# BenLangmead/bowtie2

Hardware: NVIDIA H100
Metric: Mreads/s (higher is better)
Workload: dtype u64 popcount (FM rank) + s16x2 DPX (DP)

## Files before the change

### bowtie2_b200/csrc/dp_kernels.cu

```cuda
#include "fm_device.cuh"
#include "dp_device.cuh"

#define DP_NEG (-(1 << 28))
#define DP_BIG (1 << 20)

__host__ __device__ __forceinline__ size_t dp_smem_per_warp(int maxCol) { return ((size_t)maxCol * 7 + 16 + 15) & ~(size_t)15; }

__device__ __forceinline__ int dp_max(int a, int b) { return a > b ? a : b; }

template <int R>
__device__ __forceinline__ void dp_backtrace_all(const DpLaunch &L, const bt2g_scoring &sc, const bt2g_dp_problem &p, uint64_t w,
                                                 const uint8_t *rs, const uint8_t *rq, int rdlen, const uint8_t *refw,
                                                 uint8_t *codes, bt2g_dp_cand *cands, int ncand, bt2g_dp_summary *summ,
                                                 int lane, bool local) {
	const int rdgapo = sc.rdgap_const + sc.rdgap_linear, rdgape = sc.rdgap_linear;
	const int rfgapo = sc.rfgap_const + sc.rfgap_linear, rfgape = sc.rfgap_linear;
	int SQ = rdlen >> 4; if(SQ == 0) SQ = 1;
	bt2g_dp_aln *alns = L.alns + w * (uint64_t)L.maxAlns;
	uint8_t *ops = L.ops + w * (uint64_t)L.maxAlns * L.maxOps;
	int naln = 0, flags = 0;
	auto cell = [&](int rr, int cc) -> uint8_t * { int k = rr / R; return codes + ((size_t)(cc + k) * 32 + k) * R + (rr - k * R); };
	for(int ci = 0; ci < ncand; ci++) {
		int row = cands[ci].row, col = cands[ci].col;
		const int startRow = row;
// ... 531 lines not shown
					if(c > 3) c = 5;
					bar = (i < sc.gapbar) || (rdlen[x] - 1 - i < sc.gapbar);
				}
				v[x][0] = c; v[x][1] = mm; v[x][2] = np;
				v[x][3] = bar ? -DPX_BIG : -rfgapo; v[x][4] = bar ? -DPX_BIG : -rfgape; v[x][5] = bar ? -DPX_BIG : -rdgapo;
			}
			rcP[r] = dpx_pack(v[0][0], v[1][0]); mmpP[r] = dpx_pack(v[0][1], v[1][1]); npnP[r] = dpx_pack(v[0][2], v[1][2]);
			nrfoP[r] = dpx_pack(v[0][3], v[1][3]); nrfeP[r] = dpx_pack(v[0][4], v[1][4]); nrdoP[r] = dpx_pack(v[0][5], v[1][5]);
		}
		const int lastLane0 = (rdlen[0] - 1) / R, lastLane1 = (rdlen[1] - 1) / R;
		const int lastLaneMax = lastLane0 > lastLane1 ? lastLane0 : lastLane1;
		const uint32_t nfloorP = dpx_pack(-floorv[0], -floorv[1]);

		uint32_t Hleft[R], Earr[R];
#pragma unroll
		for(int r = 0; r < R; r++) { Hleft[r] = FLOORP; Earr[r] = FLOORP; }
		uint32_t botH = FLOORP, botF = FLOORP, prevInH = FLOORP;
		const int nsteps = ncolMax + lastLaneMax;
		const size_t P4 = (size_t)(L.maxCol + 32) * 128, P1 = (size_t)(L.maxCol + 32) * 32;
		uint8_t *w4A[R / 4 + 1], *w4B[R / 4 + 1], *w1A[R % 4 + 1], *w1B[R % 4 + 1];
#pragma unroll
		for(int g = 0; g < R / 4; g++) { w4A[g] = hb[0] + g * P4 + (size_t)lane * 4; w4B[g] = hb[1] + g * P4 + (size_t)lane * 4; }
#pragma unroll
		for(int g = 0; g < R % 4; g++) { w1A[g] = hb[0] + (R / 4) * P4 + g * P1 + lane; w1B[g] = hb[1] + (R / 4) * P4 + g * P1 + lane; }
		for(int t = 0; t < nsteps; t++) {
			uint32_t inH = __shfl_up_sync(0xffffffffu, botH, 1);
			uint32_t inF = __shfl_up_sync(0xffffffffu, botF, 1);
			if(lane == 0) { inH = FLOORP; inF = FLOORP; }
			const int j = t - lane;
			if(j >= 0 && j < ncolMax && lane <= lastLaneMax) {
				const uint32_t refcP = (uint32_t)refw[0][j] | ((uint32_t)refw[1][j] << 16);
				const uint32_t refNm = ((refcP >> 2) & ONEP) * 0xffffu;
				uint32_t diag = (lane == 0) ? 0u : prevInH;
				uint32_t upH = inH, upF = inF;
				uint32_t hs[DP_RP(R)];
#pragma unroll
				for(int r = R; r < DP_RP(R); r++) hs[r] = 0u;
#pragma unroll
				for(int r = 0; r < R; r++) {
					const uint32_t F = __viaddmax_s16x2(upF, nrfeP[r], __viaddmax_s16x2(upH, nrfoP[r], FLOORP));
					const uint32_t pen = dpx_sel(refNm, npnP[r], mmpP[r]);
					const uint32_t mmask = dpx_ne01(rcP[r], refcP) * 0xffffu;
					const uint32_t Hd = __viaddmax_s16x2(diag, dpx_sel(mmask, pen, bonusP), FLOORP);
					const uint32_t E = Earr[r];
					const uint32_t H = __vimax3_s16x2(Hd, E, F);
					Earr[r] = __viaddmax_s16x2(E, nrdeP, __viaddmax_s16x2(H, nrdoP[r], FLOORP));
					hs[r] = __viaddmax_s16x2(H, nfloorP, 0u);
					diag = Hleft[r]; Hleft[r] = H;
					upH = H; upF = F;
				}
				botH = upH; botF = upF;
				prevInH = inH;
#pragma unroll
				for(int q4 = 0; q4 < R / 4; q4++) {
					const uint32_t t01 = __byte_perm(hs[4 * q4], hs[4 * q4 + 1], 0x6240), t23 = __byte_perm(hs[4 * q4 + 2], hs[4 * q4 + 3], 0x6240);
					*reinterpret_cast<uint32_t *>(w4A[q4]) = __byte_perm(t01, t23, 0x5410);
					*reinterpret_cast<uint32_t *>(w4B[q4]) = __byte_perm(t01, t23, 0x7632);
				}
#pragma unroll
				for(int g = 0; g < R % 4; g++) {
					*w1A[g] = (uint8_t)(hs[(R / 4) * 4 + g] & 0xffu);
					*w1B[g] = (uint8_t)((hs[(R / 4) * 4 + g] >> 16) & 0xffu);
				}
			} else if(j >= ncolMax) {
				botH = FLOORP; botF = FLOORP;
			}
#pragma unroll
			for(int g = 0; g < R / 4; g++) { w4A[g] += 128; w4B[g] += 128; }
#pragma unroll
			for(int g = 0; g < R % 4; g++) { w1A[g] += 32; w1B[g] += 32; }
		}
		__syncwarp();
#pragma unroll
		for(int x = 0; x < 2; x++) {
			if(!live[x]) continue;
			const int lr = rdlen[x] - 1, kk = lr / R;
			for(int j = lane; j < ncol[x]; j += 32)
				lastH[x][j] = (int)hb[x][hb_index<R>(L.maxCol + 32, lr, j)] + floorv[x];
			dp_e2e_tail<R, true>(L, sc, p[x], w[x], rs[x], rq[x], rdlen[x], ncol[x], lastH[x], candCol[x], refw[x], hb[x], L.summ + w[x], lane,
			                     DpHbPlanes<R>{hb[x], L.maxCol + 32});
		}
	}
}

#define DP_BLK_ROWS (32 * DP_BLOCK_RPL)
#define DP_BLK_HEAD 64
#define DP_BLK_MAX (DP_BLK_HEAD / 4)
static_assert(16 * 32 <= DP_BLK_MAX * DP_BLK_ROWS, "the range table must cover reads of 32 x 16 rows");

#define DP_FILL_PAD 64
__host__ __device__ __forceinline__ size_t dp_fill_smem_per_warp(int maxCol, bool offdom) {
	const size_t win = ((size_t)maxCol + 15) & ~(size_t)15;
	return 2 * (win + 2 * DP_FILL_PAD) + DP_QPROF_BYTES(DP_BLOCK_RPL) + win * (offdom ? 4 : 8);
}

template <bool B> struct DpBool { static constexpr bool value = B; };

template <typename OFF, int R, bool OFFDOM>
__global__ void __launch_bounds__(128, 8) k_dp_fill_h(DevIndex<OFF> ix, bt2g_scoring sc, DpLaunch L, uint64_t chunkStart, uint64_t chunkMax) {
	constexpr int RPL = DP_BLOCK_RPL;
	static_assert(RPL == 1 || RPL == 2, "stores are one byte or one u16 per lane and problem");
	extern __shared__ uint8_t smem[];
	const int warpInBlock = threadIdx.x >> 5, lane = threadIdx.x & 31;
	const uint64_t slot = blockIdx.x * (uint64_t)(blockDim.x >> 5) + warpInBlock;
	const uint64_t nSlots = (uint64_t)gridDim.x * (blockDim.x >> 5);
	const uint64_t nAll = L.nDev ? (uint64_t)*L.nDev : L.n;
	if(chunkStart >= nAll) return;
	const uint64_t nProb = (nAll - chunkStart < chunkMax) ? nAll - chunkStart : chunkMax;
	const uint64_t nPairs = (nProb + 1) >> 1;
	const size_t win = ((size_t)L.maxCol + 15) & ~(size_t)15;
	uint8_t *sm0 = smem + (size_t)warpInBlock * dp_fill_smem_per_warp(L.maxCol, OFFDOM);
	uint8_t *refw[2] = {sm0 + DP_FILL_PAD, sm0 + win + 3 * DP_FILL_PAD}; uint8_t *hb[2];
	for(int k = lane; k < 2 * ((int)win + 2 * DP_FILL_PAD); k += 32) sm0[k] = 4;
	uint32_t *qprof = reinterpret_cast<uint32_t *>(sm0 + 2 * (win + 2 * DP_FILL_PAD));
	uint32_t *bnd = reinterpret_cast<uint32_t *>(sm0 + 2 * (win + 2 * DP_FILL_PAD) + DP_QPROF_BYTES(RPL));
	const int rdgapo = sc.rdgap_const + sc.rdgap_linear, rdgape = sc.rdgap_linear;
	const int rfgapo = sc.rfgap_const + sc.rfgap_linear, rfgape = sc.rfgap_linear;
	const int bonus = sc.match_bonus;
	const uint32_t FLOORP = OFFDOM ? L.zeroP : dpx_both(DPX_FLOOR);
	const uint32_t nrdeP = dpx_both(-rdgape);

	for(uint64_t pw = slot; pw < nPairs; pw += nSlots) {
		uint64_t w[2] = {2 * pw, 2 * pw + 1};
		bool live[2] = {true, w[1] < nProb};
		if(!live[1]) w[1] = w[0];
		bt2g_dp_problem p[2] = {L.probs[chunkStart + w[0]], L.probs[chunkStart + w[1]]};
		hb[0] = L.codes + w[0] * L.codeStride; hb[1] = L.codes + w[1] * L.codeStride;
		uint64_t ro[2]; int rdlen[2], ncol[2], floorv[2];
		__syncwarp();
#pragma unroll
		for(int x = 0; x < 2; x++) {
			ro[x] = L.roff[p[x].read_idx];
			rdlen[x] = (int)(L.roff[p[x].read_idx + 1] - L.roff[p[x].read_idx]);
			ncol[x] = (int)(p[x].refr - p[x].refl + 1);
			floorv[x] = p[x].minsc - bonus - 1;
			if(ncol[x] <= 0 || ncol[x] > L.maxCol || rdlen[x] > 32 * R || rdlen[x] <= 0 ||
			   (int64_t)bonus * rdlen[x] - floorv[x] > 127 || floorv[x] < -DPX_LIMIT) {
				if(live[x] && lane == 0) {
					bt2g_dp_summary *sm = L.summ + chunkStart + w[x];
					sm->found = 0; sm->best = DP_NEG; sm->ncand = 0; sm->naln = 0; sm->flags = BT2G_DP_FLAG_BADSHAPE;
				}
				live[x] = false;
			}
		}
		if(!live[0] && !live[1]) continue;
		if(!live[0]) { p[0] = p[1]; ro[0] = ro[1]; rdlen[0] = rdlen[1]; ncol[0] = ncol[1]; floorv[0] = floorv[1]; }
		if(!live[1]) { p[1] = p[0]; ro[1] = ro[0]; rdlen[1] = rdlen[0]; ncol[1] = ncol[0]; floorv[1] = floorv[0]; }
		const int ncolMax = ncol[0] > ncol[1] ? ncol[0] : ncol[1];
#pragma unroll
		for(int x = 0; x < 2; x++) {
			ref_window<OFF>(ix, p[x].tidx, p[x].refl, ncol[x], refw[x], lane);
			for(int k = ncol[x] + lane; k < ncolMax; k += 32) refw[x][k] = 4;
		}
		__syncwarp();
		const int rdMax = rdlen[0] > rdlen[1] ? rdlen[0] : rdlen[1];
		const int nblk = (rdMax + DP_BLK_ROWS - 1) / DP_BLK_ROWS;
		const uint32_t nfloorP = dpx_pack(-floorv[0], -floorv[1]);
		uint32_t off = DP_BLK_HEAD;
		int plo = 0, phi = -1;

		for(int b = 0; b < nblk; b++) {
			int lo = 0, bLast = -1, nst = 0;
			if(OFFDOM && b > 0) {
				int first = -1;
				for(int c0 = plo; c0 <= phi; c0 += 32) {
					const int c = c0 + lane;
					const uint32_t m = __ballot_sync(0xffffffffu, c <= phi && bnd[c] != 0u);
					if(m) { if(first < 0) first = c0 + __ffs(m) - 1; bLast = c0 + 31 - __clz(m); }
				}
				lo = first < 0 ? 0 : first;
			}
			if(!OFFDOM || b == 0 || bLast >= 0) {
				uint32_t nrfoP[RPL], nrfeP[RPL], nrdoP[RPL];
#pragma unroll
				for(int r = 0; r < RPL; r++) {
					int v[2][3];
#pragma unroll
					for(int x = 0; x < 2; x++) {
						const int i = b * DP_BLK_ROWS + lane * RPL + r;
						bool bar = true;
						int c = 5, mm = -DPX_BIG, np = -DPX_BIG;
						if(i < rdlen[x]) {
							const int pos = p[x].fw ? i : rdlen[x] - 1 - i;
							c = L.seq[ro[x] + pos];
							c = p[x].fw ? c : (c > 3 ? 4 : 3 - c);
							int q = (int)L.qual[ro[x] + pos] - 33;
							q = q < 0 ? 0 : (q > 63 ? 63 : q);
							np = -(int)sc.npen[q];
							mm = c > 3 ? np : -(int)sc.mmpen[q];
							if(c > 3) c = 5;
							bar = (i < sc.gapbar) || (rdlen[x] - 1 - i < sc.gapbar);
						}
#pragma unroll
						for(int rf = 0; rf < 5; rf++) {
							const uint32_t pv = (uint32_t)(uint16_t)(int16_t)(rf > 3 ? np : (c == rf ? bonus : mm));
							uint32_t &q = qprof[(rf * RPL + r) * 32 + lane];
							q = x == 0 ? pv : (q | (pv << 16));
						}
						v[x][0] = bar ? -DPX_BIG : -rfgapo; v[x][1] = bar ? -DPX_BIG : -rfgape; v[x][2] = bar ? -DPX_BIG : -rdgapo;
					}
					nrfoP[r] = dpx_pack(v[0][0], v[1][0]); nrfeP[r] = dpx_pack(v[0][1], v[1][1]); nrdoP[r] = dpx_pack(v[0][2], v[1][2]);
				}
				int lastLane = (rdMax - 1 - b * DP_BLK_ROWS) / RPL;
				if(lastLane > 31) lastLane = 31;
				const bool keepBottom = b + 1 < nblk;

				const int nsteps = ncolMax - lo + lastLane;
				const int lim = lane <= lastLane ? ncolMax - lo : 0;
				auto sweep = [&](auto top) -> int {
					constexpr bool TOP = decltype(top)::value;
					constexpr int SG = 4;
					uint32_t Hleft[RPL], Earr[RPL];
#pragma unroll
					for(int r = 0; r < RPL; r++) { Hleft[r] = FLOORP; Earr[r] = FLOORP; }
					uint32_t botH = FLOORP, botF = FLOORP, prevInH = FLOORP;
					uint8_t *dA = hb[0] + off + lane * RPL, *dB = hb[1] + off + lane * RPL;
					for(int t0 = 0; t0 < nsteps; t0 += SG, dA += SG * 32 * RPL, dB += SG * 32 * RPL) {
#pragma unroll
						for(int u = 0; u < SG; u++) {
							const int t = t0 + u;
							uint32_t inH = __shfl_up_sync(0xffffffffu, botH, 1);
							uint32_t inF = __shfl_up_sync(0xffffffffu, botF, 1);
							if(TOP) {
								if(lane == 0) { inH = FLOORP; inF = FLOORP; }
							} else {
								uint32_t bh = FLOORP, bf = FLOORP;
								if(lo + t <= phi) {
									if(OFFDOM) { const uint32_t e = bnd[lo + t]; bh = __byte_perm(e, 0u, 0x4140); bf = __byte_perm(e, 0u, 0x4342); }
									else { const uint2 e = reinterpret_cast<const uint2 *>(bnd)[lo + t]; bh = e.x; bf = e.y; }
								}
								if(lane == 0) { inH = bh; inF = bf; }
							}
							const bool on = (unsigned)(t - lane) < (unsigned)lim;
							if(OFFDOM || on) {
								const int j = lo + t - lane;
								const uint32_t *qa = qprof + (int)refw[0][j] * (RPL * 32) + lane, *qb = qprof + (int)refw[1][j] * (RPL * 32) + lane;
								uint32_t diag = (TOP && lane == 0) ? (OFFDOM ? nfloorP : 0u) : prevInH;
								uint32_t upH = inH, upF = inF;
								uint32_t hs[RPL];
#pragma unroll
								for(int r = 0; r < RPL; r++) {
									const uint32_t F = __viaddmax_s16x2(upF, nrfeP[r], __viaddmax_s16x2(upH, nrfoP[r], FLOORP));
									const uint32_t sP = (qa[r * 32] & 0x0000ffffu) | (qb[r * 32] & 0xffff0000u);
									const uint32_t Hd = __viaddmax_s16x2(diag, sP, FLOORP);
									const uint32_t E = Earr[r];
									const uint32_t H = __vimax3_s16x2(Hd, E, F);
									Earr[r] = __viaddmax_s16x2(E, nrdeP, __viaddmax_s16x2(H, nrdoP[r], FLOORP));
									hs[r] = OFFDOM ? H : __viaddmax_s16x2(H, nfloorP, 0u);
									diag = Hleft[r]; Hleft[r] = H;
									upH = H; upF = F;
								}
								botH = upH; botF = upF;
								prevInH = inH;
								if(OFFDOM || on) {
									if(RPL == 2) {
										const uint32_t w2 = __byte_perm(hs[0], hs[RPL - 1], 0x6240);
										*reinterpret_cast<uint16_t *>(dA + u * 32 * RPL) = (uint16_t)w2;
										*reinterpret_cast<uint16_t *>(dB + u * 32 * RPL) = (uint16_t)(w2 >> 16);
									} else {
										dA[u * 32 * RPL] = (uint8_t)hs[0]; dB[u * 32 * RPL] = (uint8_t)(hs[0] >> 16);
									}
									if(keepBottom && lane == 31 && on) {
										if(OFFDOM) bnd[j] = __byte_perm(botH, botF, 0x6420);
										else reinterpret_cast<uint2 *>(bnd)[j] = make_uint2(botH, botF);
									}
								}
							} else {
								botH = FLOORP; botF = FLOORP;
							}
						}
						if(!TOP && OFFDOM && lo + t0 + SG - 1 >= bLast) {
							uint32_t s = botH | botF | prevInH;
#pragma unroll
							for(int r = 0; r < RPL; r++) s |= Hleft[r] | Earr[r];
							if(!__any_sync(0xffffffffu, t0 + SG - 1 - lane < lim && s != 0u)) return t0 + SG < nsteps ? t0 + SG : nsteps;
						}
					}
					return nsteps;
				};
				nst = b == 0 ? sweep(DpBool<true>()) : sweep(DpBool<false>());
			}
			if(lane == 0) {
				reinterpret_cast<uint32_t *>(hb[0])[b] = (uint32_t)lo | ((uint32_t)nst << 16);
				reinterpret_cast<uint32_t *>(hb[1])[b] = (uint32_t)lo | ((uint32_t)nst << 16);
			}
			off += (uint32_t)nst * 32 * RPL;
			plo = lo; phi = lo + nst - 32;
			if(phi > ncolMax - 1) phi = ncolMax - 1;
			__syncwarp();
		}
	}
}

struct DpHbBlocks {
	uint8_t *hb; const uint2 *tab;
	__device__ __forceinline__ uint8_t *operator()(int rr, int cc) const {
		const int k = (rr % DP_BLK_ROWS) / DP_BLOCK_RPL;
		const uint2 e = tab[rr / DP_BLK_ROWS];
		const int st = cc - (int)(e.x & 0xffffu) + k;
		return (st >= k && st < (int)(e.x >> 16)) ? hb + e.y + ((size_t)st * 32 + k) * DP_BLOCK_RPL + rr % DP_BLOCK_RPL : nullptr;
	}
};

#define DP_TAIL_SMEM_PER_WARP(maxCol, R) (dp_smem_per_warp(maxCol) + DP_PROF_BYTES(R) + DP_BLK_MAX * sizeof(uint2))

template <typename OFF, int R>
__global__ void __launch_bounds__(256) k_dp_tail_h(DevIndex<OFF> ix, bt2g_scoring sc, DpLaunch L, uint64_t chunkStart, uint64_t chunkMax) {
	extern __shared__ uint8_t smem[];
	const int warpInBlock = threadIdx.x >> 5, lane = threadIdx.x & 31;
	const uint64_t nAll = L.nDev ? (uint64_t)*L.nDev : L.n;
	if(chunkStart >= nAll) return;
	const uint64_t nProb = (nAll - chunkStart < chunkMax) ? nAll - chunkStart : chunkMax;
	const size_t perWarp = DP_TAIL_SMEM_PER_WARP(L.maxCol, R);
	int32_t *lastH = reinterpret_cast<int32_t *>(smem + (size_t)warpInBlock * perWarp);
	uint16_t *candCol = reinterpret_cast<uint16_t *>(lastH + L.maxCol);
	uint8_t *refw = reinterpret_cast<uint8_t *>(candCol + L.maxCol);
	uint8_t *prof = smem + (size_t)warpInBlock * perWarp + dp_smem_per_warp(L.maxCol);
	uint2 *tab = reinterpret_cast<uint2 *>(prof + DP_PROF_BYTES(R));
	const int bonus = sc.match_bonus;
	const uint64_t nWarps = (uint64_t)gridDim.x * (blockDim.x >> 5);
	for(uint64_t wl = blockIdx.x * (uint64_t)(blockDim.x >> 5) + warpInBlock; wl < nProb; wl += nWarps) {
		const uint64_t w = chunkStart + wl;
		const bt2g_dp_problem p = L.probs[w];
		const uint8_t *rs = L.seq + L.roff[p.read_idx], *rq = L.qual + L.roff[p.read_idx];
		const int rdlen = (int)(L.roff[p.read_idx + 1] - L.roff[p.read_idx]);
		const int ncol = (int)(p.refr - p.refl + 1);
		const int floorv = p.minsc - bonus - 1;
		__syncwarp();
		if(ncol <= 0 || ncol > L.maxCol || rdlen > 32 * R || rdlen <= 0 || (int64_t)bonus * rdlen - floorv > 127 || floorv < -DPX_LIMIT) continue;
		uint8_t *hb = L.codes + wl * L.codeStride;
		const int nblk = (rdlen + DP_BLK_ROWS - 1) / DP_BLK_ROWS;
		const uint32_t e = lane < nblk ? reinterpret_cast<const uint32_t *>(hb)[lane] : 0u;
		const uint32_t bytes = (e >> 16) * (32 * DP_BLOCK_RPL);
		uint32_t incl = bytes;
#pragma unroll
		for(int o = 1; o < 32; o <<= 1) { const uint32_t v = __shfl_up_sync(0xffffffffu, incl, o); if(lane >= o) incl += v; }
		if(lane < nblk) tab[lane] = make_uint2(e, DP_BLK_HEAD + incl - bytes);
		ref_window<OFF>(ix, p.tidx, p.refl, ncol, refw, lane);
		for(int i = lane; i < rdlen; i += 32) {
			const int pos = p.fw ? i : rdlen - 1 - i;
			int c = rs[pos]; c = p.fw ? c : (c > 3 ? 4 : 3 - c);
			int q = (int)rq[pos] - 33; q = q < 0 ? 0 : (q > 63 ? 63 : q);
			prof[i] = (uint8_t)c; prof[rdlen + i] = sc.mmpen[q]; prof[2 * rdlen + i] = sc.npen[q];
		}
		__syncwarp();
		const DpHbBlocks cell{hb, tab};
		const int lr = rdlen - 1;
		for(int j = lane; j < ncol; j += 32) { const uint8_t *c = cell(lr, j); lastH[j] = (c ? (int)*c : 0) + floorv; }
		dp_e2e_tail<R, true>(L, sc, p, w, rs, rq, rdlen, ncol, lastH, candCol, refw, hb, L.summ + w, lane, cell, prof);
	}
}

template <typename Acc>
__device__ __forceinline__ void dp_backtrace_h(const DpLaunch &L, const bt2g_scoring &sc, const bt2g_dp_problem &p, uint64_t w,
                                               const uint8_t *rs, const uint8_t *rq, int rdlen, const uint8_t *refw,
                                               const Acc &cell, bt2g_dp_cand *cands, int ncand, bt2g_dp_summary *summ, int lane,
                                               const uint8_t *prof) {
	const int rdgapo = sc.rdgap_const + sc.rdgap_linear, rdgape = sc.rdgap_linear;
	const int rfgapo = sc.rfgap_const + sc.rfgap_linear, rfgape = sc.rfgap_linear;
	const int bonus = sc.match_bonus, gapbar = sc.gapbar;
	const int vmax = bonus * rdlen - (p.minsc - bonus - 1);
	bt2g_dp_aln *alns = L.alns + w * (uint64_t)L.maxAlns;
	uint8_t *ops = L.ops + w * (uint64_t)L.maxAlns * L.maxOps;
	int naln = 0, flags = 0;
	bool screened = false;
	auto cellv = [&](int rr, int cc) -> int { const uint8_t *c = cell(rr, cc); return c ? (int)*c : 0; };
	auto rdchar = [&](int rr) -> int { const int pos = p.fw ? rr : rdlen - 1 - rr; int c = rs[pos]; return p.fw ? c : (c > 3 ? 4 : 3 - c); };
	auto rdqual = [&](int rr) -> int { const int pos = p.fw ? rr : rdlen - 1 - rr; int q = (int)rq[pos] - 33; return q < 0 ? 0 : (q > 63 ? 63 : q); };
	auto inCore = [&](int dlo, int dhi) -> bool { return dhi >= p.corel && dlo <= p.corer; };
	for(int ci = 0; ci < ncand; ci++) {
		int row = cands[ci].row, col = cands[ci].col;
		const int startRow = row, origCol = col;
		uint8_t *o = ops + (size_t)naln * L.maxOps;
		const bool room = naln < L.maxAlns;
		int nops = 0, ns = 0, gaps = 0;
		bool fail = false, core = false, done = false, first = true, filtStart = false;
		while(!done && !fail) {
			const int wd = (ci > 0 && first) ? 8 : 32;
			const int rk = row - lane, ck = col - lane;
			const bool in = lane < wd && rk >= 0 && ck >= 0;
			uint8_t *cp = in ? cell(rk, ck) : nullptr;
			const int mine = in ? (cp ? (int)*cp : 0) : 0x80;
			const int v = mine & 0x7f;
			const int vn = __shfl_down_sync(0xffffffffu, v, 1);
			int sck = 0, refc = 4; bool isN = false, isMatch = false;
			if(in) {
				refc = refw[ck];
				if(prof) {
					const int c = prof[rk];
					isN = c > 3 || refc > 3;
					isMatch = !isN && c == refc;
					sck = isN ? -(int)prof[2 * rdlen + rk] : (isMatch ? bonus : -(int)prof[rdlen + rk]);
				} else {
					const int c = rdchar(rk), q = rdqual(rk);
					isN = c > 3 || refc > 3;
					isMatch = !isN && c == refc;
					sck = isN ? -(int)sc.npen[q] : (isMatch ? bonus : -(int)sc.mmpen[q]);
				}
			}
			const bool cont = lane < wd - 1 && !(mine & 0x80) && rk > 0 && ck > 0 && vn > 0 && v == vn + sck;
			const int run = __ffs(~__ballot_sync(0xffffffffu, cont)) - 1;
			if(run > 0) {
				first = false;
				const int diagi = col - row + p.triml;
				if(inCore(diagi, diagi)) core = true;
				if(lane < run) {
					const uint8_t op = (uint8_t)((isMatch ? BT2G_OP_MATCH : BT2G_OP_MM) | (refc << 2));
					if(room && nops + lane < L.maxOps) o[nops + lane] = op;
					if(cp) *cp = (uint8_t)(mine | 0x80);
				}
				ns += __popc(__ballot_sync(0xffffffffu, lane < run && isN));
				nops += run; row -= run; col -= run;
			}
			const int endBits = __shfl_sync(0xffffffffu, mine, run);
			if(run == wd - 1 && !(endBits & 0x80) && row > 0 && col > 0) { __syncwarp(); continue; }
			if(endBits & 0x80) {
				if(first) filtStart = true;
				fail = true; break;
			}
			first = false;
			if(lane == run && cp) *cp = (uint8_t)(mine | 0x80);
			{
				const int diagi = col - row + p.triml;
				if(inCore(diagi, diagi)) core = true;
			}
			if(row == 0) { done = true; break; }
			const int cur = endBits & 0x7f;
			__syncwarp();
			int klen = 0, gapKind = 0;
			if(row >= gapbar && rdlen - 1 - row >= gapbar) {
				for(int k0 = 0; k0 < row; k0 += 32) {
					if(vmax - rfgapo - k0 * rfgape < cur) break;
					const int k = k0 + lane + 1, r2 = row - k;
					bool ok = false;
					if(r2 >= 0 && row - k + 1 >= gapbar && vmax - rfgapo - (k - 1) * rfgape >= cur) {
						const int u = cellv(r2, col) & 0x7f;
						ok = u > 0 && u - rfgapo - (k - 1) * rfgape == cur;
					}
					const uint32_t mk = __ballot_sync(0xffffffffu, ok);
					if(mk) { klen = k0 + __ffs(mk); gapKind = 1; break; }
				}
				if(gapKind == 0) {
					for(int k0 = 0; k0 < col; k0 += 32) {
						if(vmax - rdgapo - k0 * rdgape < cur) break;
						const int k = k0 + lane + 1, c2 = col - k;
						bool ok = false;
						if(c2 >= 0 && vmax - rdgapo - (k - 1) * rdgape >= cur) {
							const int u = cellv(row, c2) & 0x7f;
							ok = u > 0 && u - rdgapo - (k - 1) * rdgape == cur;
						}
						const uint32_t mk = __ballot_sync(0xffffffffu, ok);
						if(mk) { klen = k0 + __ffs(mk); gapKind = 2; break; }
					}
				}
			}
			if(gapKind == 0) { fail = true; break; }
			for(int m0 = 1; m0 < klen && !fail; m0 += 32) {
				const int mth = m0 + lane;
				uint8_t *q2 = nullptr; int b = 0;
				if(mth < klen) { q2 = gapKind == 1 ? cell(row - mth, col) : cell(row, col - mth); b = q2 ? *q2 : 0; }
				const uint32_t vm = __ballot_sync(0xffffffffu, (b & 0x80) != 0);
				const int lim = vm ? __ffs(vm) - 1 : 32;
				if(q2 && lane < lim) *q2 = (uint8_t)(b | 0x80);
				if(vm) fail = true;
			}
			if(fail) break;
			{
				const int d0 = col - row + p.triml, ni = klen - 1;
				if(ni > 0 && (gapKind == 1 ? inCore(d0 + 1, d0 + ni) : inCore(d0 - ni, d0 - 1))) core = true;
			}
			if(room) {
				for(int k = lane; k < klen; k += 32) {
					const int idx = nops + k;
					if(idx < L.maxOps) o[idx] = gapKind == 1 ? (uint8_t)BT2G_OP_REFGAP : (uint8_t)(BT2G_OP_READGAP | (refw[col - k] << 2));
				}
			}
			nops += klen; gaps += klen;
			if(gapKind == 1) row -= klen; else col -= klen;
			__syncwarp();
		}
		if(filtStart) { if(lane == 0) cands[ci].fate = BT2G_CAND_FILT_START; continue; }
		if(!fail) {
			const int c = rdchar(row), refc = refw[col];
			const bool isN = c > 3 || refc > 3;
			ns += isN;
			const uint8_t op = (uint8_t)(((!isN && c == refc) ? BT2G_OP_MATCH : BT2G_OP_MM) | (refc << 2));
			if(!core) fail = true;
			else if(ns > p.nceil) fail = true;
			else {
				if(room && lane == 0 && nops < L.maxOps) o[nops] = op;
				nops++;
			}
		}
		const bool opOverflow = nops > L.maxOps;
		if(fail) { if(lane == 0) cands[ci].fate = BT2G_CAND_FAILED; continue; }
		if(lane == 0) cands[ci].fate = BT2G_CAND_SUCCEEDED;
		if(room) {
			int refns = 0;
			for(int k = col + lane; k <= origCol; k += 32) refns += refw[k] > 3;
			refns = __reduce_add_sync(0xffffffffu, refns);
			if(lane == 0) {
				bt2g_dp_aln &a = alns[naln];
				a.cand_idx = ci; a.score = cands[ci].score; a.ns = ns; a.gaps = gaps; a.col0 = col; a.row0 = row;
				a.trim_beg = 0; a.trim_end = rdlen - 1 - startRow; a.nops = nops;
				a.refns = refns;
			}
			if(opOverflow) flags |= BT2G_DP_FLAG_OPS_OVERFLOW;
		} else {
			flags |= BT2G_DP_FLAG_ALN_OVERFLOW;
		}
		naln++;
		if(naln == 1 && !screened && ci + 1 < ncand) {
			screened = true;
			bool needSeq = false;
			for(int base = ci + 1; base < ncand; base += 32) {
				const int cj = base + lane;
				int verdict = 0;
				if(cj < ncand) {
					int r2 = cands[cj].row, c2 = cands[cj].col;
					int b = cellv(r2, c2);
					if(b & 0x80) verdict = 1;
					else {
						for(int guard = 0; guard < 4 * rdlen + 8; guard++) {
							const int curv = b & 0x7f;
							if(r2 == 0) { verdict = 2; break; }
							if(c2 > 0) {
								const int pb = cellv(r2 - 1, c2 - 1), pv = pb & 0x7f;
								const int rf = refw[c2];
								int c, mm, np;
								if(prof) { c = prof[r2]; mm = prof[rdlen + r2]; np = prof[2 * rdlen + r2]; }
								else { c = rdchar(r2); const int q = rdqual(r2); mm = sc.mmpen[q]; np = sc.npen[q]; }
								const int sc2 = (c > 3 || rf > 3) ? -np : (c == rf ? bonus : -mm);
								if(pv > 0 && curv == pv + sc2) {
									if(pb & 0x80) break;
									r2--; c2--; b = pb;
									continue;
								}
							}
							if(r2 < gapbar || rdlen - 1 - r2 < gapbar) break;
							bool moved = false, dead = false, marked = false;
							for(int k = 1; k <= r2 && r2 - k + 1 >= gapbar && vmax - rfgapo - (k - 1) * rfgape >= curv; k++) {
								const int ub = cellv(r2 - k, c2), u = ub & 0x7f;
								if(u > 0 && u - rfgapo - (k - 1) * rfgape == curv) {
									if(marked || (ub & 0x80)) dead = true; else { r2 -= k; b = ub; moved = true; }
									break;
								}
								marked = marked || (ub & 0x80);
							}
							if(!moved && !dead) {
								marked = false;
								for(int k = 1; k <= c2 && vmax - rdgapo - (k - 1) * rdgape >= curv; k++) {
									const int ub = cellv(r2, c2 - k), u = ub & 0x7f;
									if(u > 0 && u - rdgapo - (k - 1) * rdgape == curv) {
										if(marked || (ub & 0x80)) dead = true; else { c2 -= k; b = ub; moved = true; }
										break;
									}
									marked = marked || (ub & 0x80);
								}
							}
							if(!moved) break;
						}
					}
				}
				if(__any_sync(0xffffffffu, verdict == 2)) { needSeq = true; break; }
				if(cj < ncand) cands[cj].fate = verdict == 1 ? BT2G_CAND_FILT_START : BT2G_CAND_FAILED;
			}
			__syncwarp();
			if(!needSeq) break;
		}
	}
	if(lane == 0) { summ->naln = naln; summ->flags |= flags; }
}

template <typename K>
static unsigned dp_resident_grid(K kernel, int threads, size_t smem, uint64_t numSlots, int warpsPerBlock) {
	int dev = 0, sms = 148, nb = 1;
	cudaGetDevice(&dev);
	cudaDeviceGetAttribute(&sms, cudaDevAttrMultiProcessorCount, dev);
	if(cudaOccupancyMaxActiveBlocksPerMultiprocessor(&nb, kernel, threads, smem) != cudaSuccess || nb < 1) nb = 1;
	uint64_t g = (uint64_t)nb * sms, cap = numSlots / warpsPerBlock;
	return (unsigned)(g < cap ? g : cap);
}

template <typename OFF, int R>
static void launch_dp_e2e_r(const DevIndex<OFF> &ix, const bt2g_scoring &sc, const DpLaunch &L, cudaStream_t st) {
	const int warpsPerBlock = 4;
	if(L.packed == 3) {
		int dev = 0, sms = 148; cudaGetDevice(&dev); cudaDeviceGetAttribute(&sms, cudaDevAttrMultiProcessorCount, dev);
		const size_t smF = (size_t)warpsPerBlock * dp_fill_smem_per_warp(L.maxCol, sc.match_bonus == 0);
		const size_t smT = (size_t)8 * DP_TAIL_SMEM_PER_WARP(L.maxCol, R);
		auto kfill = sc.match_bonus == 0 ? k_dp_fill_h<OFF, R, true> : k_dp_fill_h<OFF, R, false>;
		if(smF > 48 * 1024) cudaFuncSetAttribute(kfill, cudaFuncAttributeMaxDynamicSharedMemorySize, (int)smF);
		if(smT > 48 * 1024) cudaFuncSetAttribute(k_dp_tail_h<OFF, R>, cudaFuncAttributeMaxDynamicSharedMemorySize, (int)smT);
		int nbF = 1, nbT = 1;
		if(cudaOccupancyMaxActiveBlocksPerMultiprocessor(&nbF, kfill, warpsPerBlock * 32, smF) != cudaSuccess || nbF < 1) nbF = 1;
		if(cudaOccupancyMaxActiveBlocksPerMultiprocessor(&nbT, k_dp_tail_h<OFF, R>, 256, smT) != cudaSuccess || nbT < 1) nbT = 1;
		auto mark = [&]() { if(L.tev && L.tevN && *L.tevN < L.tevCap) cudaEventRecord(L.tev[(*L.tevN)++], st); };
		mark();
		for(uint64_t c0 = 0; c0 < L.n; c0 += L.chunk) {
			kfill<<<(unsigned)(nbF * sms), warpsPerBlock * 32, smF, st>>>(ix, sc, L, c0, L.chunk);
			mark();
			k_dp_tail_h<OFF, R><<<(unsigned)(nbT * sms), 256, smT, st>>>(ix, sc, L, c0, L.chunk);
			mark();
		}
	} else if(L.packed == 2) {
		const size_t smem = (size_t)warpsPerBlock * 2 * dp_smem_per_warp(L.maxCol);
		if(smem > 48 * 1024) cudaFuncSetAttribute(k_dp_e2e_h<OFF, R>, cudaFuncAttributeMaxDynamicSharedMemorySize, (int)smem);
		const unsigned grid = dp_resident_grid(k_dp_e2e_h<OFF, R>, warpsPerBlock * 32, smem, L.numSlots, warpsPerBlock);
		k_dp_e2e_h<OFF, R><<<grid, warpsPerBlock * 32, smem, st>>>(ix, sc, L);
	} else if(L.packed) {
		const size_t smem = (size_t)warpsPerBlock * 2 * dp_smem_per_warp(L.maxCol);
		if(smem > 48 * 1024) cudaFuncSetAttribute(k_dp_e2e_x2<OFF, R>, cudaFuncAttributeMaxDynamicSharedMemorySize, (int)smem);
		const unsigned grid = dp_resident_grid(k_dp_e2e_x2<OFF, R>, warpsPerBlock * 32, smem, L.numSlots, warpsPerBlock);
		k_dp_e2e_x2<OFF, R><<<grid, warpsPerBlock * 32, smem, st>>>(ix, sc, L);
	} else {
		const size_t smem = (size_t)warpsPerBlock * dp_smem_per_warp(L.maxCol);
		if(smem > 48 * 1024) cudaFuncSetAttribute(k_dp_e2e<OFF, R>, cudaFuncAttributeMaxDynamicSharedMemorySize, (int)smem);
		const unsigned grid = dp_resident_grid(k_dp_e2e<OFF, R>, warpsPerBlock * 32, smem, L.numSlots, warpsPerBlock);
		k_dp_e2e<OFF, R><<<grid, warpsPerBlock * 32, smem, st>>>(ix, sc, L);
	}
}

template <typename OFF>
int launch_dp_e2e(const DevIndex<OFF> &ix, const bt2g_scoring &sc, const DpLaunch &L, int maxRdLen, cudaStream_t st) {
	if(L.n == 0) return 0;
	switch(dp_rows_per_lane(maxRdLen, L.packed)) {
		case 4: launch_dp_e2e_r<OFF, 4>(ix, sc, L, st); break;
		case 5: launch_dp_e2e_r<OFF, 5>(ix, sc, L, st); break;
		case 6: launch_dp_e2e_r<OFF, 6>(ix, sc, L, st); break;
		case 8: launch_dp_e2e_r<OFF, 8>(ix, sc, L, st); break;
		case 10: launch_dp_e2e_r<OFF, 10>(ix, sc, L, st); break;
		case 12: launch_dp_e2e_r<OFF, 12>(ix, sc, L, st); break;
		case 16: launch_dp_e2e_r<OFF, 16>(ix, sc, L, st); break;
		default: return -1;
	}
	return 0;
}
template int launch_dp_e2e<uint32_t>(const DevIndex<uint32_t> &, const bt2g_scoring &, const DpLaunch &, int, cudaStream_t);
template int launch_dp_e2e<uint64_t>(const DevIndex<uint64_t> &, const bt2g_scoring &, const DpLaunch &, int, cudaStream_t);

template <typename OFF, int R>
__global__ void __launch_bounds__(128) k_dp_local(DevIndex<OFF> ix, bt2g_scoring sc, DpLaunch L) {
	extern __shared__ uint8_t smem[];
	const int warpInBlock = threadIdx.x >> 5, lane = threadIdx.x & 31;
	const uint64_t slot = blockIdx.x * (uint64_t)(blockDim.x >> 5) + warpInBlock;
	const uint64_t nSlots = (uint64_t)gridDim.x * (blockDim.x >> 5);
	const uint64_t nProb = L.nDev ? (uint64_t)*L.nDev : L.n;
	const size_t perWarp = dp_smem_per_warp(L.maxCol);
	int32_t *wsm = reinterpret_cast<int32_t *>(smem + (size_t)warpInBlock * perWarp);
	uint8_t *refw = reinterpret_cast<uint8_t *>(wsm + L.maxCol) + 2 * (size_t)L.maxCol;
	uint8_t *codes = L.codes + slot * L.codeStride;
	uint64_t *raw = L.rawKeys + slot * (uint64_t)L.maxRaw;
	const int rdgapo = sc.rdgap_const + sc.rdgap_linear, rdgape = sc.rdgap_linear;
	const int rfgapo = sc.rfgap_const + sc.rfgap_linear, rfgape = sc.rfgap_linear;
	const int bonus = sc.match_bonus;

	for(uint64_t w = slot; w < nProb; w += nSlots) {
		const bt2g_dp_problem p = L.probs[w];
		const uint8_t *rs = L.seq + L.roff[p.read_idx];
		const uint8_t *rq = L.qual + L.roff[p.read_idx];
		const int rdlen = (int)(L.roff[p.read_idx + 1] - L.roff[p.read_idx]);
		const int ncol = (int)(p.refr - p.refl + 1);
		bt2g_dp_summary *summ = L.summ + w;
		__syncwarp();
		if(ncol <= 0 || ncol + 1 > L.maxCol || rdlen > 32 * R || rdlen <= 0 || bonus <= 0) {
			if(lane == 0) { summ->found = 0; summ->best = DP_NEG; summ->ncand = 0; summ->naln = 0; summ->flags = BT2G_DP_FLAG_BADSHAPE; }
			continue;
		}
		for(int k = lane; k <= ncol; k += 32) refw[k] = (uint8_t)ref_base<OFF>(ix, p.tidx, p.refl + k);
		if(lane == 0) wsm[0] = 0;
		__syncwarp();

		int rc[R + 1], mmp[R], npn[R];
		bool bar[R];
#pragma unroll
		for(int r = 0; r <= R; r++) {
			int i = lane * R + r;
			int c = 6;
			if(i < rdlen) {
				int pos = p.fw ? i : rdlen - 1 - i;
				c = rs[pos];
				c = p.fw ? c : (c > 3 ? 4 : 3 - c);
				if(r < R) {
					int q = (int)rq[pos] - 33;
					q = q < 0 ? 0 : (q > 63 ? 63 : q);
					npn[r] = sc.npen[q];
					mmp[r] = c > 3 ? npn[r] : sc.mmpen[q];
					bar[r] = (i < sc.gapbar) || (rdlen - 1 - i < sc.gapbar);
				}
			} else if(r < R) { mmp[r] = 0; npn[r] = 0; bar[r] = true; }
			rc[r] = c;
		}
		const int lastLane = (rdlen - 1) / R;
		const int minrow = (int)(((int64_t)p.minsc + bonus - 1) / bonus) - 1;

		int Hleft[R], Earr[R], Eprev[R];
#pragma unroll
		for(int r = 0; r < R; r++) { Hleft[r] = 0; Earr[r] = 0; Eprev[r] = 0; }
		int botH = 0, botF = 0, prevInH = 0, lmax = 0;
		const int nsteps = ncol + lastLane;
		for(int t = 0; t < nsteps; t++) {
			int inH = __shfl_up_sync(0xffffffffu, botH, 1);
			int inF = __shfl_up_sync(0xffffffffu, botF, 1);
			if(lane == 0) { inH = 0; inF = 0; }
			const int j = t - lane;
			if(j >= 0 && j < ncol && lane <= lastLane) {
				const int refc = refw[j], refn = refw[j + 1];
				const bool refN = refc > 3;
				int diag = (lane == 0) ? 0 : prevInH;
				int upH = inH, upF = inF;
				uint32_t packed[(R + 3) / 4];
#pragma unroll
				for(int q4 = 0; q4 < (R + 3) / 4; q4++) packed[q4] = 0;
#pragma unroll
				for(int r = 0; r < R; r++) {
					const int i = lane * R + r;
					const int fo = upH - rfgapo, fe = upF - rfgape;
					int F = bar[r] ? 0 : dp_max(dp_max(fo, fe), 0);
					const int fsel = (upH > 0 && fo == F) ? 1 : ((upF > 0 && fe == F) ? 2 : 0);
					int s = (rc[r] == refc && !refN) ? bonus : -mmp[r];
					s = (refN || rc[r] > 3) ? -npn[r] : s;
					const int Hd = diag + s;
					const int E = Earr[r];
					const int H = dp_max(__vimax3_s32(Hd, E, F), 0);
					int hsel = 0;
					if(diag > 0 && H == Hd) hsel = 1;
					else if(!bar[r]) {
						if(upH > 0 && H == fo) hsel = 2;
						else if(upF > 0 && H == fe) hsel = 3;
						else if(Hleft[r] > 0 && H == Hleft[r] - rdgapo) hsel = 4;
						else if(Eprev[r] > 0 && H == Eprev[r] - rdgape) hsel = 5;
					}
					const int esel = (Hleft[r] > 0 && Hleft[r] - rdgapo == E) ? 1 : ((Eprev[r] > 0 && Eprev[r] - rdgape == E) ? 2 : 0);
					const uint32_t code = (uint32_t)(hsel | (esel << 3) | (fsel << 5));
					packed[r >> 2] |= code << ((r & 3) * 8);
					const int eo = bar[r] ? 0 : H - rdgapo, ee = E - rdgape;
					if(i < rdlen && i >= minrow && H >= p.minsc && rc[r] == refc && !(i < rdlen - 1 && rc[r + 1] == refn)) {
						const int pos = atomicAdd(&wsm[0], 1);
						if(pos < L.maxRaw) raw[pos] = ((uint64_t)(uint32_t)H << 32) | ((uint64_t)i << 16) | (uint64_t)j;
					}
					lmax = dp_max(lmax, i < rdlen ? H : 0);
					diag = Hleft[r]; Hleft[r] = H; Eprev[r] = E; Earr[r] = dp_max(dp_max(eo, ee), 0);
					upH = H; upF = F;
				}
				botH = upH; botF = upF;
				prevInH = inH;
				uint8_t *dst = codes + ((size_t)t * 32 + lane) * R;
				if(R == 4) *reinterpret_cast<uint32_t *>(dst) = packed[0];
				else if(R == 8) *reinterpret_cast<uint2 *>(dst) = make_uint2(packed[0], packed[1]);
				else {
#pragma unroll
					for(int q4 = 0; q4 < (R + 3) / 4; q4++) reinterpret_cast<uint32_t *>(dst)[q4] = packed[q4];
				}
			} else if(j >= ncol) {
				botH = 0; botF = 0;
			}
		}
		__syncwarp();
		int best = lmax;
#pragma unroll
		for(int o = 16; o > 0; o >>= 1) best = dp_max(best, __shfl_xor_sync(0xffffffffu, best, o));
		if(lane == 0) { summ->best = best; summ->flags = 0; summ->naln = 0; summ->ncand = 0; summ->found = 0; }
		if(best < p.minsc) continue;
		const int nrawAll = wsm[0];
		const int nraw = nrawAll < L.maxRaw ? nrawAll : L.maxRaw;
		bt2g_dp_cand *cands = L.cands + w * (uint64_t)L.maxCands;
		for(int a0 = 0; a0 < nraw; a0 += 32) {
			const int a = a0 + lane;
			if(a < nraw) {
				const uint64_t key = raw[a];
				int rank = 0;
				for(int k = 0; k < nraw; k++) rank += raw[k] > key;
				if(rank < L.maxCands) {
					cands[rank].score = (int32_t)(key >> 32); cands[rank].row = (int32_t)((key >> 16) & 0xffff);
					cands[rank].col = (int32_t)(key & 0xffff); cands[rank].fate = 0;
				}
			}
		}
		const int ncand = nraw < L.maxCands ? nraw : L.maxCands;
		if(lane == 0) {
			summ->ncand = nrawAll; summ->found = nrawAll > 0;
			if(nrawAll > L.maxCands || nrawAll > L.maxRaw) summ->flags |= BT2G_DP_FLAG_CAND_OVERFLOW;
		}
		__syncwarp();
		dp_backtrace_all<R>(L, sc, p, w, rs, rq, rdlen, refw, codes, cands, ncand, summ, lane, true);
	}
}

template <typename OFF>
int launch_dp_local(const DevIndex<OFF> &ix, const bt2g_scoring &sc, const DpLaunch &L, int maxRdLen, cudaStream_t st) {
	if(L.n == 0) return 0;
	const int warpsPerBlock = 4;
	const size_t perWarp = dp_smem_per_warp(L.maxCol);
	size_t smem = (size_t)warpsPerBlock * perWarp;
	unsigned grid = (unsigned)(L.numSlots / warpsPerBlock);
	if(maxRdLen <= 128) {
		if(smem > 48 * 1024) cudaFuncSetAttribute(k_dp_local<OFF, 4>, cudaFuncAttributeMaxDynamicSharedMemorySize, (int)smem);
		k_dp_local<OFF, 4><<<grid, warpsPerBlock * 32, smem, st>>>(ix, sc, L);
	} else if(maxRdLen <= 256) {
		if(smem > 48 * 1024) cudaFuncSetAttribute(k_dp_local<OFF, 8>, cudaFuncAttributeMaxDynamicSharedMemorySize, (int)smem);
		k_dp_local<OFF, 8><<<grid, warpsPerBlock * 32, smem, st>>>(ix, sc, L);
	} else if(maxRdLen <= 512) {
		if(smem > 48 * 1024) cudaFuncSetAttribute(k_dp_local<OFF, 16>, cudaFuncAttributeMaxDynamicSharedMemorySize, (int)smem);
		k_dp_local<OFF, 16><<<grid, warpsPerBlock * 32, smem, st>>>(ix, sc, L);
	} else {
		return -1;
	}
	return 0;
}
template int launch_dp_local<uint32_t>(const DevIndex<uint32_t> &, const bt2g_scoring &, const DpLaunch &, int, cudaStream_t);
template int launch_dp_local<uint64_t>(const DevIndex<uint64_t> &, const bt2g_scoring &, const DpLaunch &, int, cudaStream_t);
```

Baseline: 2.754.

## Rework DP tail kernel: warp-parallel candidate selection, dynamic work claiming, skip empty problems

New measurement: 2.800 (median of 6 runs). 1.02x the previous value.

```diff
diff --git a/bowtie2_b200/csrc/dp_kernels.cu b/bowtie2_b200/csrc/dp_kernels.cu
--- a/bowtie2_b200/csrc/dp_kernels.cu
+++ b/bowtie2_b200/csrc/dp_kernels.cu
@@ -857,52 +857,151 @@
 	}
 };
 
-#define DP_TAIL_SMEM_PER_WARP(maxCol, R) (dp_smem_per_warp(maxCol) + DP_PROF_BYTES(R) + DP_BLK_MAX * sizeof(uint2))
+__host__ __device__ __forceinline__ int dp_tail_key_cap(int maxCands, int maxCol) {
+	const int n = maxCands < maxCol ? maxCands : maxCol;
+	int c = 1;
+	while(c < n) c <<= 1;
+	return c;
+}
+__host__ __device__ __forceinline__ size_t dp_tail_win_bytes(int maxCol) { return ((size_t)maxCol + 15) & ~(size_t)15; }
+__host__ __device__ __forceinline__ size_t dp_tail_smem_per_warp(int maxCol, int maxCands, int R) {
+	return (dp_tail_win_bytes(maxCol) + DP_PROF_BYTES(R) + DP_BLK_MAX * sizeof(uint2) + (size_t)dp_tail_key_cap(maxCands, maxCol) * 4 + 15) &
+	       ~(size_t)15;
+}
+__host__ __device__ __forceinline__ unsigned *dp_tail_claim(const DpLaunch &L) { return reinterpret_cast<unsigned *>(L.codes + L.codeStride) - 1; }
+
+__device__ __forceinline__ int dp_tail_cands(const DpLaunch &L, const bt2g_dp_problem &p, const uint8_t *hb, const uint2 *tab, int rdlen,
+                                             int ncol, int floorv, uint32_t *keys, bt2g_dp_cand *cands, bt2g_dp_summary *summ, int lane) {
+	const int lr = rdlen - 1, k = (lr % DP_BLK_ROWS) / DP_BLOCK_RPL;
+	const uint2 e = tab[lr / DP_BLK_ROWS];
+	const int lo = (int)(e.x & 0xffffu), steps = (int)(e.x >> 16);
+	const int hi = lo + steps - k < ncol ? lo + steps - k : ncol;
+	const uint8_t *row = hb + e.y + (size_t)k * 33 * DP_BLOCK_RPL + lr % DP_BLOCK_RPL;
+	auto key = [&](int c) -> uint32_t { return c < hi ? (uint32_t)row[(size_t)(c - lo) * 32 * DP_BLOCK_RPL] << 16 | (uint32_t)c : 0u; };
+	const uint32_t thr = (uint32_t)(p.minsc - floorv) << 16;
+	const uint32_t below = (1u << lane) - 1u;
+	uint32_t kmax = 0;
+	int total = 0;
+	for(int c0 = lo; c0 < hi; c0 += 32) {
+		const uint32_t x = key(c0 + lane);
+		kmax = x > kmax ? x : kmax;
+		const uint32_t m = __ballot_sync(0xffffffffu, x >= thr);
+		const int slot = total + __popc(m & below);
+		if(x >= thr && slot < L.maxCands) keys[slot] = x;
+		total += __popc(m);
+	}
+	kmax = __reduce_max_sync(0xffffffffu, kmax);
+	const int best = (int)(kmax >> 16) + floorv;
+	if(lane == 0) {
+		summ->best = best; summ->naln = 0; summ->ncand = total; summ->found = total > 0;
+		summ->flags = total > L.maxCands ? BT2G_DP_FLAG_CAND_OVERFLOW : 0;
+	}
+	if(total > L.maxCands) {
+		uint32_t tlo = thr, thi = 128u << 16;
+		while(thi - tlo > 1) {
+			const uint32_t mid = tlo + (thi - tlo) / 2;
+			int cnt = 0;
+			for(int c0 = lo; c0 < hi; c0 += 32) cnt += key(c0 + lane) >= mid;
+			if(__reduce_add_sync(0xffffffffu, cnt) >= L.maxCands) tlo = mid; else thi = mid;
+		}
+		int kept = 0;
+		for(int c0 = lo; c0 < hi; c0 += 32) {
+			const uint32_t x = key(c0 + lane);
+			const uint32_t m = __ballot_sync(0xffffffffu, x >= tlo);
+			if(x >= tlo) keys[kept + __popc(m & below)] = x;
+			kept += __popc(m);
+		}
+	}
+	const int n = total < L.maxCands ? total : L.maxCands;
+	__syncwarp();
+	auto put = [&](int i, uint32_t x) {
+		bt2g_dp_cand &cd = cands[i];
+		cd.score = (int)(x >> 16) + floorv; cd.col = (int)(x & 0xffffu); cd.row = lr; cd.fate = 0;
+	};
+	if(n <= 32) {
+		uint32_t x = lane < n ? keys[lane] : 0u;
+#pragma unroll
+		for(int size = 2; size <= 32; size <<= 1) {
+#pragma unroll
+			for(int j = size >> 1; j > 0; j >>= 1) {
+				const uint32_t y = __shfl_xor_sync(0xffffffffu, x, j);
+				const bool desc = (lane & size) == 0, first = (lane & j) == 0;
+				x = (first == desc) ? (x > y ? x : y) : (x < y ? x : y);
+			}
+		}
+		if(lane < n) put(lane, x);
+	} else {
+		int P = 64;
+		while(P < n) P <<= 1;
+		for(int i = n + lane; i < P; i += 32) keys[i] = 0u;
+		__syncwarp();
+		for(int size = 2; size <= P; size <<= 1) {
+			for(int j = size >> 1; j > 0; j >>= 1) {
+				for(int i = lane; i < P / 2; i += 32) {
+					const int a = ((i & ~(j - 1)) << 1) | (i & (j - 1)), b = a + j;
+					const uint32_t x = keys[a], y = keys[b];
+					if((a & size) == 0 ? x < y : x > y) { keys[a] = y; keys[b] = x; }
+				}
+				__syncwarp();
+			}
+		}
+		for(int i = lane; i < n; i += 32) put(i, keys[i]);
+	}
+	__syncwarp();
+	return n;
+}
 
 template <typename OFF, int R>
-__global__ void __launch_bounds__(256) k_dp_tail_h(DevIndex<OFF> ix, bt2g_scoring sc, DpLaunch L, uint64_t chunkStart, uint64_t chunkMax) {
+__global__ void __launch_bounds__(256, 4) k_dp_tail_h(DevIndex<OFF> ix, bt2g_scoring sc, DpLaunch L, uint64_t chunkStart, uint64_t chunkMax) {
 	extern __shared__ uint8_t smem[];
 	const int warpInBlock = threadIdx.x >> 5, lane = threadIdx.x & 31;
 	const uint64_t nAll = L.nDev ? (uint64_t)*L.nDev : L.n;
 	if(chunkStart >= nAll) return;
 	const uint64_t nProb = (nAll - chunkStart < chunkMax) ? nAll - chunkStart : chunkMax;
-	const size_t perWarp = DP_TAIL_SMEM_PER_WARP(L.maxCol, R);
-	int32_t *lastH = reinterpret_cast<int32_t *>(smem + (size_t)warpInBlock * perWarp);
-	uint16_t *candCol = reinterpret_cast<uint16_t *>(lastH + L.maxCol);
-	uint8_t *refw = reinterpret_cast<uint8_t *>(candCol + L.maxCol);
-	uint8_t *prof = smem + (size_t)warpInBlock * perWarp + dp_smem_per_warp(L.maxCol);
+	uint8_t *refw = smem + (size_t)warpInBlock * dp_tail_smem_per_warp(L.maxCol, L.maxCands, R);
+	uint8_t *prof = refw + dp_tail_win_bytes(L.maxCol);
 	uint2 *tab = reinterpret_cast<uint2 *>(prof + DP_PROF_BYTES(R));
+	uint32_t *keys = reinterpret_cast<uint32_t *>(tab + DP_BLK_MAX);
 	const int bonus = sc.match_bonus;
-	const uint64_t nWarps = (uint64_t)gridDim.x * (blockDim.x >> 5);
-	for(uint64_t wl = blockIdx.x * (uint64_t)(blockDim.x >> 5) + warpInBlock; wl < nProb; wl += nWarps) {
+	unsigned *next = dp_tail_claim(L);
+	unsigned wl = 0;
+	if(lane == 0) wl = atomicAdd(next, 1u);
+	wl = __shfl_sync(0xffffffffu, wl, 0);
+	while(wl < nProb) {
+		unsigned nx = 0;
+		if(lane == 0) nx = atomicAdd(next, 1u);
 		const uint64_t w = chunkStart + wl;
+		uint8_t *hb = L.codes + (uint64_t)wl * L.codeStride;
+		const uint32_t e = lane < DP_BLK_MAX ? reinterpret_cast<const uint32_t *>(hb)[lane] : 0u;
 		const bt2g_dp_problem p = L.probs[w];
 		const uint8_t *rs = L.seq + L.roff[p.read_idx], *rq = L.qual + L.roff[p.read_idx];
 		const int rdlen = (int)(L.roff[p.read_idx + 1] - L.roff[p.read_idx]);
 		const int ncol = (int)(p.refr - p.refl + 1);
 		const int floorv = p.minsc - bonus - 1;
 		__syncwarp();
-		if(ncol <= 0 || ncol > L.maxCol || rdlen > 32 * R || rdlen <= 0 || (int64_t)bonus * rdlen - floorv > 127 || floorv < -DPX_LIMIT) continue;
-		uint8_t *hb = L.codes + wl * L.codeStride;
-		const int nblk = (rdlen + DP_BLK_ROWS - 1) / DP_BLK_ROWS;
-		const uint32_t e = lane < nblk ? reinterpret_cast<const uint32_t *>(hb)[lane] : 0u;
-		const uint32_t bytes = (e >> 16) * (32 * DP_BLOCK_RPL);
-		uint32_t incl = bytes;
-#pragma unroll
-		for(int o = 1; o < 32; o <<= 1) { const uint32_t v = __shfl_up_sync(0xffffffffu, incl, o); if(lane >= o) incl += v; }
-		if(lane < nblk) tab[lane] = make_uint2(e, DP_BLK_HEAD + incl - bytes);
-		ref_window<OFF>(ix, p.tidx, p.refl, ncol, refw, lane);
-		for(int i = lane; i < rdlen; i += 32) {
-			const int pos = p.fw ? i : rdlen - 1 - i;
-			int c = rs[pos]; c = p.fw ? c : (c > 3 ? 4 : 3 - c);
-			int q = (int)rq[pos] - 33; q = q < 0 ? 0 : (q > 63 ? 63 : q);
-			prof[i] = (uint8_t)c; prof[rdlen + i] = sc.mmpen[q]; prof[2 * rdlen + i] = sc.npen[q];
-		}
-		__syncwarp();
-		const DpHbBlocks cell{hb, tab};
-		const int lr = rdlen - 1;
-		for(int j = lane; j < ncol; j += 32) { const uint8_t *c = cell(lr, j); lastH[j] = (c ? (int)*c : 0) + floorv; }
-		dp_e2e_tail<R, true>(L, sc, p, w, rs, rq, rdlen, ncol, lastH, candCol, refw, hb, L.summ + w, lane, cell, prof);
+		if(!(ncol <= 0 || ncol > L.maxCol || rdlen > 32 * R || rdlen <= 0 || (int64_t)bonus * rdlen - floorv > 127 || floorv < -DPX_LIMIT)) {
+			const int nblk = (rdlen + DP_BLK_ROWS - 1) / DP_BLK_ROWS;
+			const uint32_t bytes = (e >> 16) * (32 * DP_BLOCK_RPL);
+			uint32_t incl = bytes;
+#pragma unroll
+			for(int o = 1; o < 32; o <<= 1) { const uint32_t v = __shfl_up_sync(0xffffffffu, incl, o); if(lane >= o) incl += v; }
+			if(lane < nblk) tab[lane] = make_uint2(e, DP_BLK_HEAD + incl - bytes);
+			__syncwarp();
+			bt2g_dp_cand *cands = L.cands + w * (uint64_t)L.maxCands;
+			const int ncand = dp_tail_cands(L, p, hb, tab, rdlen, ncol, floorv, keys, cands, L.summ + w, lane);
+			if(ncand > 0) {
+				ref_window<OFF>(ix, p.tidx, p.refl, ncol, refw, lane);
+				for(int i = lane; i < rdlen; i += 32) {
+					const int pos = p.fw ? i : rdlen - 1 - i;
+					int c = rs[pos]; c = p.fw ? c : (c > 3 ? 4 : 3 - c);
+					int q = (int)rq[pos] - 33; q = q < 0 ? 0 : (q > 63 ? 63 : q);
+					prof[i] = (uint8_t)c; prof[rdlen + i] = sc.mmpen[q]; prof[2 * rdlen + i] = sc.npen[q];
+				}
+				__syncwarp();
+				dp_backtrace_h(L, sc, p, w, rs, rq, rdlen, refw, DpHbBlocks{hb, tab}, cands, ncand, L.summ + w, lane, prof);
+			}
+		}
+		wl = __shfl_sync(0xffffffffu, nx, 0);
 	}
 }
 
@@ -1143,7 +1242,7 @@
 	if(L.packed == 3) {
 		int dev = 0, sms = 148; cudaGetDevice(&dev); cudaDeviceGetAttribute(&sms, cudaDevAttrMultiProcessorCount, dev);
 		const size_t smF = (size_t)warpsPerBlock * dp_fill_smem_per_warp(L.maxCol, sc.match_bonus == 0);
-		const size_t smT = (size_t)8 * DP_TAIL_SMEM_PER_WARP(L.maxCol, R);
+		const size_t smT = (size_t)8 * dp_tail_smem_per_warp(L.maxCol, L.maxCands, R);
 		auto kfill = sc.match_bonus == 0 ? k_dp_fill_h<OFF, R, true> : k_dp_fill_h<OFF, R, false>;
 		if(smF > 48 * 1024) cudaFuncSetAttribute(kfill, cudaFuncAttributeMaxDynamicSharedMemorySize, (int)smF);
 		if(smT > 48 * 1024) cudaFuncSetAttribute(k_dp_tail_h<OFF, R>, cudaFuncAttributeMaxDynamicSharedMemorySize, (int)smT);
@@ -1153,6 +1252,7 @@
 		auto mark = [&]() { if(L.tev && L.tevN && *L.tevN < L.tevCap) cudaEventRecord(L.tev[(*L.tevN)++], st); };
 		mark();
 		for(uint64_t c0 = 0; c0 < L.n; c0 += L.chunk) {
+			cudaMemsetAsync(dp_tail_claim(L), 0, sizeof(unsigned), st);
 			kfill<<<(unsigned)(nbF * sms), warpsPerBlock * 32, smF, st>>>(ix, sc, L, c0, L.chunk);
 			mark();
 			k_dp_tail_h<OFF, R><<<(unsigned)(nbT * sms), 256, smT, st>>>(ix, sc, L, c0, L.chunk);
```
